# kyoungseoun-chung/pyapes

Hardware: AMD Instinct MI355X
Metric: cell-updates*iters/sec, 3-D Poisson CG (higher is better)
Workload: dtype f64; 1 GPU; 3-D Poisson 512x512x512 double, periodic BCs, CG (BASELINE config 3); global_cells=134217728, parallelism=single

## Files before the change

### pyapes_amd/csrc/pa_bc.hip

```cpp
#include "pa_host.h"

#include <math.h>
#include <stdlib.h>
#include <stdio.h>
#include <string.h>

#include <algorithm>
#include <new>

template <typename T>
struct BCArgs {
  int axis, side, type;
  T sval;
  const T* vals;
  T c23, dxf, ndir;
  T c43, c13;
  const T* far0;
  const T* far1;
  const int* done;
};

template <typename T>
__global__ void __launch_bounds__(PA_BLOCK) k_bc_face(DevGeom G, T* __restrict__ x, BCArgs<T> B) {
  if (B.done && *B.done) return;
// ... 346 lines not shown
    T t1 = B.c43 * x[base + (p1 - off) * st];
    T t2 = B.c13 * x[base + (p2 - off) * st];
    t1 = t1 - t2;
    return t1 + ct;
  }
  if (B.type == 3) return x[base + (p1 - off) * st];
  if (lower) {
    T vp = x[base + (1 - off) * st];
    T vf = B.far0 ? B.far0[q] : x[base + (N - 1 - off) * st];
    T vff = B.far0 ? B.far1[q] : x[base + (N - 2 - off) * st];
    T t1 = vp - vf;
    return t1 + vff;
  }
  if (B.far0) {
    T t1 = B.far0[q] - x[base + (N - 1 - off) * st];
    return t1 + x[base + (N - 2 - off) * st];
  }
  return x0_new;
}

template <typename T>
__global__ void __launch_bounds__(PA_BLOCK) k_bc_pair(DevGeom G, T* __restrict__ x, BCPairArgs<T> P,
                                                       const int* __restrict__ done, T* __restrict__ shell_old,
                                                       double* __restrict__ partials, int mode) {
  if (done && *done) return;
  const int a = P.axis;
  const int64_t nu = (a == 0) ? G.n1 : G.n0;
  const int64_t nv = (a == 2) ? G.n1 : G.n2;
  const int64_t N = (a == 0) ? G.g0 : (a == 1 ? G.n1 : G.n2);
  const int64_t off = (a == 0) ? G.off0 : 0;
  const int64_t st = (a == 0) ? G.s0 : (a == 1 ? G.s1 : 1);
  double s[1] = {0.0};
  for (int64_t q = (int64_t)blockIdx.x * blockDim.x + threadIdx.x; q < nu * nv;
       q += (int64_t)gridDim.x * blockDim.x) {
    const int64_t u = q / nv, v = q - u * nv;
    int64_t base;
    bool owned = true;
    if (a == 0) {
      base = u * G.s1 + v;
      if (G.act[1] && (u == 0 || u == G.n1 - 1)) owned = false;
      if (G.act[2] && (v == 0 || v == G.n2 - 1)) owned = false;
    } else if (a == 1) {
      base = u * G.s0 + v;
      if (G.act[2] && (v == 0 || v == G.n2 - 1)) owned = false;
    } else {
      base = u * G.s0 + v * G.s1;
    }
    T x0_new = (T)0;
    if (P.lo.type) {
      T* xf = x + base + (0 - off) * st;
      T val;
      if (mode == 3) {
        val = *xf;
      } else {
        val = pa_bc_face_value<T>(P.lo, x, base, st, off, N, q, (T)0);
        *xf = val;
      }
      x0_new = val;
// ... 13 lines not shown
      T val;
      if (mode == 3) {
        val = *xf;
      } else {
        val = pa_bc_face_value<T>(P.hi, x, base, st, off, N, q, x0_new);
        *xf = val;
      }
      if (mode && owned) {
        if (mode == 1) {
          T df = val - shell_old[P.pos_hi + q];
          T p = df * df;
          s[0] += (double)p;
        }
        shell_old[P.pos_hi + q] = val;
      }
    }
  }
  if (mode == 1) pa_block_reduce_store<1>(s, partials);
}

template <typename T>
static int pa_bc_shell_fused(pa_ctx* c, T* x, double* part2, int with_delta, bool guarded, int* nsh, bool standalone);
template <typename T>
static int pa_bc_pair_apply(pa_ctx* c, T* x, double* part2, int mode, bool guarded, int* nsh);
template <typename T>
static void pa_shell_launch(pa_ctx* c, const T* x, T* shell, double* part2, int with_delta);

template <typename T>
int pa_bc_apply_faces(pa_ctx* c, T* x, bool guarded) {
  const DevGeom& G = c->G;
  for (int w = 0; w < c->nbc; ++w) {
    int f = c->bc_order[w];
    const HostBC& b = c->bc[f];
    if (b.type == PA_BC_NONE) continue;
    int a = f >> 1, side = f & 1;
    if (!G.act[a]) continue;
    if (a == 0) {
      if (side == 0 && G.off0 != 0) continue;
      if (side == 1 && G.off0 + G.n0 != G.g0) continue;
    }
    BCArgs<T> B;
    memset(&B, 0, sizeof(B));
    B.axis = a; B.side = side; B.type = b.type;
    B.vals = (const T*)b.vals;
    B.c43 = (T)(4.0 / 3.0);
    B.c13 = (T)(1.0 / 3.0);
    B.c23 = (T)(2.0 / 3.0);
// ... 199 lines not shown
    if (side == 0 && G.off0 != 0) B.type = 0;
    if (side == 1 && G.off0 + G.n0 != G.g0) B.type = 0;
  }
  B.vals = (const T*)b.vals;
  B.c43 = (T)(4.0 / 3.0);
  B.c13 = (T)(1.0 / 3.0);
  B.c23 = (T)(2.0 / 3.0);
  B.dxf = (T)b.dxf;
  B.ndir = side == 0 ? (T)-1 : (T)1;
  B.done = guarded ? pa_done_flag(c) : nullptr;
  if (b.type == PA_BC_DIRICHLET) B.sval = (T)b.value;
  if (b.type == PA_BC_NEUMANN) {
    T pre = (T)((2.0 / 3.0) * b.value);
    pre = pre * B.dxf;
    pre = pre * B.ndir;
    B.sval = pre;
  }
  if (b.type == PA_BC_PERIODIC && a == 0 && G.n0 != G.g0) {
    B.far0 = (const T*)(side == 0 ? c->bc_far_lo0 : c->bc_far_hi0);
    B.far1 = (const T*)c->bc_far_lo1;
  }
}

template <typename T>
static int pa_bc_pair_apply(pa_ctx* c, T* x, double* part2, int mode, bool guarded, int* nsh) {
  const DevGeom& G = c->G;
  const int64_t sz[3] = {G.n1 * G.n2, G.n0 * G.n2, G.n0 * G.n1};
  int64_t start[6], total = 0;
  for (int f = 0; f < 6; ++f) { start[f] = total; total += G.act[f >> 1] ? sz[f >> 1] : 0; }
  T* shell = (T*)c->scr[SCR_SHELL];
  int rows = 0;
  for (int a = 0; a < 3; ++a) {
    if (!G.act[a]) continue;
    BCPairArgs<T> P;
    bc_face_args<T>(c, 2 * a, P.lo, guarded);
    bc_face_args<T>(c, 2 * a + 1, P.hi, guarded);
    if (mode != 3 && ((P.lo.type == PA_BC_PERIODIC && a == 0 && G.n0 != G.g0 && !P.lo.far0) ||
                      (P.hi.type == PA_BC_PERIODIC && a == 0 && G.n0 != G.g0 && !P.hi.far0))) {
      pa_set_err(c, "periodic axis-0 BC on a slab needs the far planes (pa_slab_set)");
      return PA_E_STATE;
    }
    if (!P.lo.type && !P.hi.type) continue;
    P.axis = a;
    P.pos_lo = start[2 * a];
    P.pos_hi = start[2 * a + 1];
    const int nb = pa_grid_blocks(sz[a]);
    hipLaunchKernelGGL(k_bc_pair<T>, dim3(nb), dim3(PA_BLOCK), 0, c->stream, G, x, P,
                       guarded ? pa_done_flag(c) : (const int*)nullptr, shell, part2 ? part2 + rows : nullptr,
                       mode);
    if (mode == 1) rows += nb;
  }
  if (nsh) *nsh = rows;
  PA_HIP(c, hipGetLastError());
  return PA_OK;
}


int pa_bc_shell_rows(const pa_ctx* c) {
  if (c->bc_fused || !c->bc_pair) return pa_shell_blocks(c);
  const DevGeom& G = c->G;
  const int64_t sz[3] = {G.n1 * G.n2, G.n0 * G.n2, G.n0 * G.n1};
  int rows = 0;
  for (int a = 0; a < 3; ++a) {
    if (!G.act[a]) continue;
    int lo = c->bc[2 * a].type, hi = c->bc[2 * a + 1].type;
    if (a == 0) {
      if (G.off0 != 0) lo = 0;
      if (G.off0 + G.n0 != G.g0) hi = 0;
    }
    if (lo || hi) rows += pa_grid_blocks(sz[a]);
  }
  return rows;
}

template <typename T>
static void pa_shell_launch(pa_ctx* c, const T* x, T* shell, double* part2, int with_delta) {
  hipLaunchKernelGGL(k_shell<T>, dim3(pa_shell_blocks(c)), dim3(PA_BLOCK), 0, c->stream, c->G, c->sc, x, shell, part2,
                     with_delta);
}

void pa_bc_plan(pa_ctx* c) {
  c->bc_static = pa_bc_is_static(c);
  c->bc_fused = pa_bc_fusable(c);
  c->bc_pair = (!c->bc_fused && pa_bc_pairable(c)) ? 1 : 0;
  c->shell_cur = 0;
}

template <typename T>
int pa_bc_fill_start(pa_ctx* c, T* x, bool filled_by_driver) {
  if (c->bc_fused && !filled_by_driver)
    return pa_bc_shell_fused<T>(c, x, nullptr, 0, false, nullptr, false);
  if (c->bc_pair) return pa_bc_pair_apply<T>(c, x, nullptr, filled_by_driver ? 3 : 2, false, nullptr);
  if (!filled_by_driver)
    if (int rc = pa_bc_apply_faces<T>(c, x)) return rc;
  pa_shell_launch<T>(c, (const T*)x, (T*)c->scr[SCR_SHELL], (double*)c->scr[SCR_PART2], 0);
  return PA_OK;
}

template <typename T>
int pa_bc_fill_step(pa_ctx* c, T* x, double* part2, int* nsh) {
  *nsh = 0;
  if (c->bc_static) return PA_OK;
  if (c->bc_fused) return pa_bc_shell_fused<T>(c, x, part2, 1, true, nsh, false);
  if (c->bc_pair) return pa_bc_pair_apply<T>(c, x, part2, 1, true, nsh);
  if (int rc = pa_bc_apply_faces<T>(c, x, true)) return rc;
  *nsh = pa_shell_blocks(c);
  pa_shell_launch<T>(c, (const T*)x, (T*)c->scr[SCR_SHELL], part2, 1);
  return PA_OK;
}

#define PA_BC_INST(T)                                                                            \
  template int pa_bc_apply_faces<T>(pa_ctx*, T*, bool);                                          \
  template int pa_bc_apply_auto<T>(pa_ctx*, T*, bool);                                           \
  template int pa_bc_fill_start<T>(pa_ctx*, T*, bool);                                           \
  template int pa_bc_fill_step<T>(pa_ctx*, T*, double*, int*);
PA_BC_INST(float)
PA_BC_INST(double)
#undef PA_BC_INST
```

### pyapes_amd/csrc/pa_cg3d.hip

```cpp
#include "pa_cg3d_kernel.h"
#include "pa_cg2d_kernel.h"

template <typename T>
int pa_cg3d_phase_a(pa_ctx* c, const DevEq<T>& E, Vec<T> r, Vec<T> d, T* dnew, double* partials) {
  const int mode = c->cg_pitch ? 3 : cg3d_mode<T>(c, E, {r.p, d.p, dnew, r.glo, r.ghi, d.glo, d.ghi}, false, false, true);
  if (!mode) return 0;
  const bool rz = c->coord == PA_COORD_RZ;
  Cg3dArgs<T> A;
  memset(&A, 0, sizeof(A));
  fill_common<T>(c, E, A);
  A.ps1 = c->cg_ps1; A.ps0 = c->cg_ps1 * c->G.n1;
  A.r = r; A.d = d; A.dnew = dnew; A.partials = partials;
  A.reverse = 0;
  if (c->fold_b_n > 0) {
    A.pre_part = c->fold_b_part;
    A.pre_n = c->fold_b_n;
    A.pre_shell = c->fold_b_shell ? c->fold_b_shell : (const double*)c->scr[SCR_PART2];
    A.pre_nsh = c->fold_b_nsh;
    A.sc_w = c->sc_alt;
    A.pre_sums = pa_sums(c);
  }
  int n = (mode == 1 || mode == 3 || mode == 4) ? launch_cg2d<T, 0>(c, A, mode == 3) : 0;
  if (n == 0 && rz) return 0;
  if (n == 0) n = launch_any<T, 0>(c, A, mode);
// ... 7 lines not shown
}

template <typename T>
int pa_cg3d_phase_b(pa_ctx* c, const DevEq<T>& E, Vec<T> d, T* x, T* r, double* partials) {
  T* const r_out = c->cg_r_out ? (T*)c->cg_r_out : r;
  const int mode = c->cg_pitch ? 3 : cg3d_mode<T>(c, E, {d.p, x, r, r_out, d.glo, d.ghi, c->r_send_lo, c->r_send_hi}, false, false, true);
  if (!mode) return 0;
  const bool rz = c->coord == PA_COORD_RZ;
  Cg3dArgs<T> A;
  memset(&A, 0, sizeof(A));
  fill_common<T>(c, E, A);
  A.ps1 = c->cg_ps1; A.ps0 = c->cg_ps1 * c->G.n1;
  A.d = d; A.x = x; A.rw = r; A.rw_out = r_out; A.partials = partials;
  if (!c->slab_fold_live) {
    A.send_lo = (T*)c->r_send_lo; A.send_hi = (T*)c->r_send_hi;
  }
  A.reverse = 1;
  if (c->fold_a_n > 0) {
    A.pre_part = (const double*)c->scr[SCR_PART] + 2 * (size_t)PA_MAX_PARTIALS;
    A.pre_n = c->fold_a_n;
    A.sc_w = c->sc;
    A.pre_sums = pa_sums(c);
  }
  int n = (mode == 1 || mode == 3 || mode == 4) ? launch_cg2d<T, 1>(c, A, mode == 3) : 0;
  if (n == 0 && rz) return 0;
  if (n == 0) n = launch_any<T, 1>(c, A, mode);
  if (n > 0 && hipGetLastError() != hipSuccess) { pa_set_err(c, "k_cg3d phase B launch failed"); return PA_E_HIP; }
  if (n > 0) c->fold_a_n = 0;
  return n;
}

template <typename T>
int pa_tile3d_jacobi(pa_ctx* c, const DevEq<T>& E, Vec<T> x, const T* rhs, T* xnew, double omega, double* partials) {
  const int mode = cg3d_mode<T>(c, E, {x.p, rhs, xnew, x.glo, x.ghi}, false, false, true);
  if (!mode) return 0;
  const bool rz = c->coord == PA_COORD_RZ;
  Cg3dArgs<T> A;
  memset(&A, 0, sizeof(A));
  fill_common<T>(c, E, A);
  A.d = x; A.out = xnew; A.aux = rhs; A.p0 = (T)omega; A.partials = partials;
  if (c->fold_b_n > 0) {
    A.pre_part = c->fold_b_part;
    A.pre_n = c->fold_b_n;
    A.pre_shell = c->fold_b_shell ? c->fold_b_shell : (const double*)c->scr[SCR_PART2];
    A.pre_nsh = c->fold_b_nsh;
    A.sc_w = c->sc_alt;
    A.pre_sums = pa_sums(c);
  }
  int n = 0;
  if (mode == 1 || mode == 4) {
    const bool back2 = c->jac_alt && c->jac_dir && !c->plan_only;
// ... 25 lines not shown
```

### pyapes_amd/csrc/pa_cg3d_kernel.h

```cpp
#pragma once
#include "pa_host.h"

#include <stdio.h>
#include <stdlib.h>
#include <string.h>

template <typename T> struct VecOf;
template <> struct VecOf<double> { static constexpr int N = 2; typedef double type __attribute__((ext_vector_type(2))); };
template <> struct VecOf<float>  { static constexpr int N = 4; typedef float type __attribute__((ext_vector_type(4))); };

template <typename T>
struct Cg3dArgs {
  DevGeom G;
  LapCoef<T> lap;
  T coeff, sign;
  int has_coeff;
  const T* coeff_f;
  const SolverScalars* sc;
  Vec<T> r, d;
  T* dnew;
  T* x;
  T* rw;
  T* rw_out;
  T* send_lo;
// ... 10 lines not shown
  int lap_off;
  GradCoef<T> grd;
  int gnd;
  int64_t ps0, ps1;
  const T* rz;
  int64_t rz_n;
  int interior_only;
  int out_all;
  int bcl_type[6];
  T bcl_val[6];
  T bcl_c43, bcl_c13;
  const double* pre_part;
  const double* pre_shell;
  int pre_n, pre_nsh;
  SolverScalars* sc_w;
  double* pre_sums;
  const T* stg_phi0;
  T stg_c0, stg_c1;
  const T* src;
  T src_val;
  const T* vel_f[3];
  T vel_v[3];
  int vel_own;
};

__device__ __forceinline__ int pa_xcd_remap(int b, int nb) {
  const int q = nb >> 3, r = nb & 7, xcd = b & 7, w = b >> 3;
  return (xcd < r ? xcd * (q + 1) : r * (q + 1) + (xcd - r) * q) + w;
}

__device__ __forceinline__ int64_t pa_wrapmod(int64_t v, int64_t n) {
  v %= n;
  return v < 0 ? v + n : v;
}

template <typename T, int RJ, int PHASE, bool CF = false, int KIND = 0, int LAY = 0, bool STG = false>
__global__ void __launch_bounds__(256) k_cg3d(Cg3dArgs<T> A) {
  static_assert(!STG || PHASE == 3, "STG: the explicit Euler step");
  constexpr int PH = PHASE == 9 ? 4 : PHASE;
  constexpr bool NARROW = LAY == 1, PITCH = LAY == 2;
  static_assert(!PITCH || ((PH == 0 || PH == 1 || PH == 5 || PH == 6 || PH == 8) && !CF && KIND == 0),
                "PITCH: the CG / BiCGSTAB phases of a plain Laplacian");
  constexpr int VEC = NARROW ? 1 : VecOf<T>::N;
  typedef T V __attribute__((ext_vector_type(VEC)));
  constexpr int TJ = 4 * RJ, TK = 64 * VEC, TKP = TK + 2 * VEC;
  __shared__ __attribute__((aligned(16))) T tile[2][TJ + 2][TKP];

  (void)sizeof(int[PH >= 0 && PH <= 8 ? 1 : -1]);
  T beta = (T)0, alpha = (T)0;
  T omega = (T)0;
  const DevGeom& G = A.G;
  const int lane = threadIdx.x & 63, wv = threadIdx.x >> 6;
  const int vb = pa_xcd_remap(blockIdx.x, gridDim.x);
  const int tiles = A.tiles_j * A.tiles_k;
  const int chunk = vb / tiles, tl = vb - chunk * tiles;
  const int tjb = tl / A.tiles_k, tkb = tl - tjb * A.tiles_k;
  const int64_t i0 = (int64_t)chunk * G.n0 / A.chunks, i1 = (int64_t)(chunk + 1) * G.n0 / A.chunks;
  const int CI = (int)(i1 - i0);
  const int64_t j0 = (int64_t)tjb * TJ, k0 = (int64_t)tkb * TK;
  constexpr int rev = (PHASE == 1 || PHASE == 9) ? 1 : 0;

  const int64_t kg = k0 + (int64_t)lane * VEC;
  const int64_t kc = pa_wrapmod(kg, G.n2);
  const bool kvalid = kg < G.n2;
  const int64_t fs0 = PITCH ? A.ps0 : G.s0, fs1 = PITCH ? A.ps1 : G.s1;
  const int64_t kcf = PITCH ? (kg < fs1 ? kg : 0) : kc;
  int64_t jrow[RJ];
  unsigned rowS = 0, rowShell = 0, rowValid = 0, rowLo = 0, rowHi = 0;
#pragma unroll
  for (int jj = 0; jj < RJ; ++jj) {
    const int64_t jg = j0 + wv * RJ + jj;
    jrow[jj] = pa_wrapmod(jg, G.n1);
    const bool valid = jg < G.n1;
    if (valid) rowValid |= 1u << jj;
    if (valid && jg >= G.slo[1] && jg <= G.shi[1]) rowS |= 1u << jj;
    if (jg == 0 || jg == G.n1 - 1) rowShell |= 1u << jj;
    const int rc = pa_row_case(G, 1, jg, G.n1, G.treat);
    if (rc == 1) rowLo |= 1u << jj;
    if (rc == 2) rowHi |= 1u << jj;
  }
  unsigned rowPLo = 0, rowPHi = 0, colPLo = 0, colPHi = 0;
  if (PH == 3 || PH == 7 || KIND != 0) {
#pragma unroll
    for (int jj = 0; jj < RJ; ++jj) {
      const int64_t jg = j0 + wv * RJ + jj;
      if (G.bct[2] == 4 && jg == 1) rowPLo |= 1u << jj;
      if (G.bct[3] == 4 && jg == G.n1 - 2) rowPHi |= 1u << jj;
    }
#pragma unroll
    for (int v = 0; v < VEC; ++v) {
      if (G.bct[4] == 4 && kg + v == 1) colPLo |= 1u << v;
      if (G.bct[5] == 4 && kg + v == G.n2 - 2) colPHi |= 1u << v;
    }
  }
  unsigned colS = 0, colShell = 0, colLo = 0, colHi = 0;
#pragma unroll
  for (int v = 0; v < VEC; ++v) {
    const int64_t kk = kg + v;
    if (kvalid && kk >= G.slo[2] && kk <= G.shi[2]) colS |= 1u << v;
    if (kk == 0 || kk == G.n2 - 1) colShell |= 1u << v;
    const int rc = pa_row_case(G, 2, kk, G.n2, G.treat);
    if (rc == 1) colLo |= 1u << v;
    if (rc == 2) colHi |= 1u << v;
  }
#ifdef PA_PLAIN_EXPERIMENT
  rowLo = rowHi = colLo = colHi = 0;
  rowS = rowValid = (1u << RJ) - 1;
  colS = (1u << VEC) - 1;
#endif
  const int64_t hrow = (wv == 0) ? pa_wrapmod(j0 - 1, G.n1) : pa_wrapmod(j0 + TJ, G.n1);
  const bool hvec = (wv == 0 || wv == 3);
  const bool hsc = (wv == 1 && lane < 2 * TJ);
  const int hs_row = lane >> 1, hs_side = lane & 1;
  const int64_t hs_off = pa_wrapmod(j0 + hs_row, G.n1) * fs1 +
                         (hs_side ? pa_wrapmod(k0 + TK, G.n2) : pa_wrapmod(k0 - 1, G.n2));

  auto plane_of = [&](int q) -> int64_t { return rev ? (i1 - 1 - q) : (i0 + q); };
  auto pptr = [&](const Vec<T>& v, int64_t ii) -> const T* {
    return ii < 0 ? v.glo : (ii >= G.n0 ? v.ghi : v.p + ii * fs0);
  };

  struct Raw {
    V d[RJ];
    V r[RJ];
    V q[RJ];
    V hd, hr, hq;
// ... 650 lines not shown
        } else if (PH == 0) {
          const T e = inS ? xc : (T)0;
          outd[v] = e;
          T p = e * res[jj][v];
          s0 += (double)p;
        } else {
          const T xo = xv[jj][v];
          T ad = alpha * xc;
          T xn = xo + ad;
          T aAd = alpha * res[jj][v];
          T rn = rv[jj][v] - aAd;
          xn = inS ? xn : xo;
          rn = inS ? rn : (T)0;
          T p = rn * rn;
          s0 += (double)p;
          const bool offshell = inS && !(iShell || (rowShell >> jj & 1) || (colShell >> v & 1));
          T df = xn - xo;
          T p2 = df * df;
          s1 += offshell ? (double)p2 : 0.0;
          outd[v] = rn;
          outx[v] = xn;
        }
      }
      if (kvalid && (rowValid >> jj & 1)) {
        const int64_t o = ii * G.s0 + jrow[jj] * G.s1 + kc;
        const int64_t ob = PITCH ? ii * fs0 + jrow[jj] * fs1 + kcf : o;
        if (PH == 8) {
          *reinterpret_cast<V*>(A.out2 + ob) = outx;
        } else if (PH == 5 || PH == 6) {
          if (PH == 5 || A.out) *reinterpret_cast<V*>(A.out + ob) = outd;
          *reinterpret_cast<V*>(A.out2 + ob) = outx;
        } else if (PH >= 2) {
          *reinterpret_cast<V*>(A.out + o) = outd;
        } else if (PH == 0) {
          if (PITCH) __builtin_nontemporal_store(outd, reinterpret_cast<V*>(A.dnew + ii * fs0 + jrow[jj] * fs1 + kcf));
          else if (NARROW) *reinterpret_cast<V*>(A.dnew + o) = outd;
          else __builtin_nontemporal_store(outd, reinterpret_cast<V*>(A.dnew + o));
        } else {
          if (PITCH) {
            __builtin_nontemporal_store(outd, reinterpret_cast<V*>(A.rw_out + ii * fs0 + jrow[jj] * fs1 + kcf));
            T* xp = A.x + ii * G.s0 + jrow[jj] * G.s1;
#pragma unroll
            for (int v = 0; v < VEC; ++v)
              if (kg + v < G.n2) xp[kg + v] = outx[v];
          } else if (NARROW) {
            *reinterpret_cast<V*>(A.x + o) = outx;
// ... 70 lines not shown
  if (c->ndim != 3 && c->ndim != 2) return 0;
  int il, id;
  if (!eq_lap_div<T>(E, il, id, field_speed) || (id >= 0 && !allow_div)) return 0;
  if ((c->ndim == 3 && c->G.n0 < 3) || c->G.n1 < 3 || c->G.n2 < 3) return 0;
  uintptr_t bits = il >= 0 ? (uintptr_t)E.t[il].coeff_f : 0;
  if (id >= 0) bits |= (uintptr_t)E.t[id].u_f;
  for (const void* q : ptrs) bits |= (uintptr_t)q;
  if (bits & (sizeof(T) - 1)) return 0;
  constexpr int VEC = VecOf<T>::N;
  if ((bits & 15) || c->G.n2 % VEC != 0 || c->G.n2 < 2 * VEC) return 2;
  return 1;
}

static int cus_of(pa_ctx* c) {
  static int cus = 0;
  if (!cus) {
    hipDeviceProp_t prop;
    if (hipGetDeviceProperties(&prop, c->device) == hipSuccess) cus = prop.multiProcessorCount;
    if (cus <= 0) cus = 256;
  }
  return cus;
}

template <typename T, int RJ, int PHASE, bool CF, int KIND = 0, int LAY = 0, bool STG = false>
static int blocks_per_cu() {
  static int cached = 0;
  if (!cached) {
    int n = 0;
    if (hipOccupancyMaxActiveBlocksPerMultiprocessor(&n, k_cg3d<T, RJ, PHASE, CF, KIND, LAY, STG>, 256, 0) != hipSuccess || n <= 0) n = 2;
    cached = n;
  }
  return cached;
}

template <typename T, int RJ, int PHASE, bool CF = false, int KIND = 0, int LAY = 0, bool STG = false>
static int launch_cg3d(pa_ctx* c, Cg3dArgs<T>& A) {
  constexpr bool NARROW = LAY == 1;
  constexpr int VEC = NARROW ? 1 : VecOf<T>::N;
  constexpr int TJ = 4 * RJ, TK = 64 * VEC;
  const DevGeom& G = c->G;
  int64_t n1e = G.n1, n2e = G.n2;
  if (PHASE == 0 || PHASE == 1 || PHASE == 5 || PHASE == 6 || PHASE == 8) {
    if (G.bct[3] != PA_BC_PERIODIC && n1e > 2) n1e -= 1;
    if (G.bct[5] != PA_BC_PERIODIC && n2e > 2) n2e -= 1;
  }
  A.tiles_j = (int)((n1e + TJ - 1) / TJ);
  A.tiles_k = (int)((n2e + TK - 1) / TK);
  const int tiles = A.tiles_j * A.tiles_k;
  const int capacity = cus_of(c) * blocks_per_cu<T, RJ, PHASE, CF, KIND, LAY, STG>();
  int chunks = capacity / tiles;
  if (chunks < 1) chunks = 1;
  if (chunks > G.n0) chunks = (int)G.n0;
  if (c->chunks > 0 && chunks > c->chunks) chunks = c->chunks;
  A.chunks = chunks;
  const int nblk = tiles * chunks;
  if (nblk > PA_MAX_PARTIALS) return 0;
  static int dbg = -1;
  if (dbg < 0) dbg = getenv("PYAPES_HIP_DEBUG") ? 8 : 0;
  if (dbg > 0) {
    --dbg;
    fprintf(stderr, "[pyapes_hip] k_cg3d phase %c%s%s: tiles %dx%d chunks %d (CI ~%lld) blocks %d, %d blocks/CU x %d CUs\n",
            (char)('A' + PHASE), LAY == 1 ? " (narrow)" : (LAY == 2 ? " (pitched)" : ""), STG ? " (RK stage)" : "", A.tiles_j, A.tiles_k, chunks, (long long)(G.n0 / chunks), nblk,
            blocks_per_cu<T, RJ, PHASE, CF, KIND, LAY, STG>(), cus_of(c));
  }
  if (c->plan_only) return nblk;
  hipLaunchKernelGGL((k_cg3d<T, RJ, PHASE, CF, KIND, LAY, STG>), dim3(nblk), dim3(256), 0, c->stream, A);
  return nblk;
}

template <typename T, int PHASE = 0>
static int pick_rj(pa_ctx* c, bool narrow = false, bool cg_phase = false) {
  const int VEC = narrow ? 1 : VecOf<T>::N;
  const DevGeom& G = c->G;
  if (!G.act[0]) return 4;
  const int64_t n1e = G.n1 - ((cg_phase && G.bct[3] != PA_BC_PERIODIC && G.n1 > 2) ? 1 : 0);
  const int64_t n2e = G.n2 - ((cg_phase && G.bct[5] != PA_BC_PERIODIC && G.n2 > 2) ? 1 : 0);
  const int64_t tk = (n2e + 64 * VEC - 1) / (64 * VEC);
  const int cap = cus_of(c) * 2;
  auto chunk_len = [&](int rj) {
    const int64_t tiles = ((n1e + 4 * rj - 1) / (4 * rj)) * tk;
    const int64_t chunks = cap / tiles > 0 ? cap / tiles : 1;
    return G.n0 / chunks;
  };
  if (PHASE == 3) {
    return chunk_len(4) >= 12 ? 4 : 2;
  }
  if (G.n1 <= 4) return 1;
  if (G.n1 <= 8) return 2;
  return (chunk_len(4) < 24 && chunk_len(2) >= 24) ? 2 : 4;
// ... 26 lines not shown
      PA_EULER_CASE(PA_OP_DIV_UPWIND_COMPAT)
      PA_EULER_CASE(PA_OP_DIV_UPWIND)
      default: return 0;
    }
#undef PA_EULER_CASE
  }
  if constexpr (PHASE == 2 || PHASE == 5 || PHASE == 6 || PHASE == 8) {
    if (A.kind != 0) {
      const bool four = pick_rj<T>(c, NARROW == 1) == 4;
#define PA_DIV_CASE(K)                                                                   \
      case K:                                                                            \
        return four ? launch_cg3d<T, 4, PHASE, false, K, NARROW>(c, A)                   \
                    : launch_cg3d<T, 2, PHASE, false, K, NARROW>(c, A);
      switch (A.kind) {
        PA_DIV_CASE(PA_OP_DIV_CENTRAL)
        PA_DIV_CASE(PA_OP_DIV_UPWIND_COMPAT)
        PA_DIV_CASE(PA_OP_DIV_UPWIND)
        default: return 0;
      }
#undef PA_DIV_CASE
    }
  }
  const int rj = pick_rj<T>(c, NARROW == 1, PHASE == 0 || PHASE == 1 || PHASE == 5 || PHASE == 6 || PHASE == 8);
  switch (rj) {
    case 1: return launch_cg3d<T, 1, PHASE, false, 0, NARROW>(c, A);
    case 2: return launch_cg3d<T, 2, PHASE, false, 0, NARROW>(c, A);
    default: return launch_cg3d<T, 4, PHASE, false, 0, NARROW>(c, A);
  }
}

template <typename T, int PHASE>
static int launch_pitched(pa_ctx* c, Cg3dArgs<T>& A) {
  static_assert(PHASE == 0 || PHASE == 1 || PHASE == 5 || PHASE == 6 || PHASE == 8, "PITCH: CG / BiCGSTAB phases");
  if (A.coeff_f || A.kind != 0) return 0;
  switch (pick_rj<T>(c, false, true)) {
    case 1: return launch_cg3d<T, 1, PHASE, false, 0, 2>(c, A);
    case 2: return launch_cg3d<T, 2, PHASE, false, 0, 2>(c, A);
    default: return launch_cg3d<T, 4, PHASE, false, 0, 2>(c, A);
  }
}

template <typename T, int PHASE, bool STG = false>
static int launch_any(pa_ctx* c, Cg3dArgs<T>& A, int mode) {
  if constexpr (PHASE == 0 || PHASE == 1 || PHASE == 5 || PHASE == 6 || PHASE == 8) {
    if (mode == 3) return launch_pitched<T, PHASE>(c, A);
  }
// ... 41 lines not shown
```

### pyapes_amd/csrc/pa_core.hip

```cpp
#include "pa_host.h"

#include <dlfcn.h>
#include <math.h>
#include <stdlib.h>
#include <stdio.h>
#include <string.h>

#include <algorithm>
#include <chrono>
#include <new>

template <typename T>
__global__ void __launch_bounds__(PA_BLOCK) k_rz_tables(int64_t nr, const T* __restrict__ r_nodes, T dr,
                                                         T* __restrict__ tab) {
  auto nn = [](T v) -> T { return (isnan(v) || isinf(v)) ? (T)0 : v; };
  const T h2 = dr * dr;
  const T c23 = (T)(2.0 / 3.0), c13 = (T)(1.0 / 3.0);
  for (int64_t i = (int64_t)blockIdx.x * blockDim.x + threadIdx.x; i < nr; i += (int64_t)gridDim.x * blockDim.x) {
    const T r = r_nodes[i];
    T t = (T)2 * r;
    const T s = nn(dr / t);
    T ap = (T)1 + s;
    T am = (T)1 - s;
    tab[i] = ap / h2;
// ... 267 lines not shown

int pa_ctx_set_option(pa_ctx* c, const char* name, int value) {
  if (!c || !name) return PA_E_ARG;
  if (c->solve != PA_SOLVE_NONE) { pa_set_err(c, "pa_ctx_set_option during a solve"); return PA_E_STATE; }
  if (!strcmp(name, "fastpath")) c->fastpath = value != 0;
  else if (!strcmp(name, "sf")) c->sf = (value == 2 || value == 4) ? value : (value != 0);
  else if (!strcmp(name, "chunks")) c->chunks = value < 0 ? 0 : value;
  else if (!strcmp(name, "vself")) c->vself = value != 0;
  else if (!strcmp(name, "sfq")) c->sfq = value < 0 ? 0 : value;
  else if (!strcmp(name, "fold")) c->fold = value != 0;
  else if (!strcmp(name, "resident")) c->resident = value != 0;
  else if (!strcmp(name, "cg2d_mincells")) c->cg2d_mincells = value;
  else if (!strcmp(name, "bcl")) c->bcl = value != 0;
  else if (!strcmp(name, "pitch")) c->pitch = value != 0;
  else if (!strcmp(name, "place")) c->place = value != 0;
  else if (!strcmp(name, "place_minbytes")) c->ps.minbytes = value < 0 ? 0 : (size_t)value;
  else if (!strcmp(name, "place_blocks")) c->ps.blocks = value < 0 ? 0 : (value > PA_PLACE_MAXSPARE ? PA_PLACE_MAXSPARE : value);
  else if (!strcmp(name, "place_budget")) c->ps.budget = 0.01 * (value < 0 ? 0 : value);
  else if (!strcmp(name, "resident_coop")) c->resident_coop = value != 0;
  else if (!strcmp(name, "bc_path")) c->bc_path = value & 7;
  else if (!strcmp(name, "bicg_pfold")) c->bicg_pfold = value != 0;
  else if (!strcmp(name, "bicg_srv")) c->bicg_srv = value != 0;
  else if (!strcmp(name, "jac_alt")) c->jac_alt = value != 0;
  else if (!strcmp(name, "rhs_full")) c->rhs_full = value != 0;
  else if (!strcmp(name, "res_cells")) c->res_cells = value;
  else if (!strcmp(name, "res_nt")) c->res_nt = value;
  else if (!strcmp(name, "res_nt_cells")) c->res_nt_cells = value;
  else if (!strcmp(name, "res_spin")) c->res_spin = value;
  else if (!strcmp(name, "res_rzlean")) c->res_rzlean = value != 0;
  else if (!strcmp(name, "comm")) c->opt_comm = value != 0;
  else if (!strcmp(name, "slab_fold")) c->opt_slab_fold = value != 0;
  else if (!strcmp(name, "comm_overlap")) c->comm_overlap = value < 0 ? -1 : (value != 0);
  else if (!strcmp(name, "comm_timeout")) c->comm_timeout = value > 0 ? value : 60;
  else if (!strcmp(name, "roctx")) { g_roctx.want = value != 0; g_roctx.state = 0; }
  else { pa_set_err(c, "pa_ctx_set_option: unknown option '%s'", name); return PA_E_ARG; }
  return PA_OK;
}

int pa_ctx_get_option(const pa_ctx* c, const char* name, int* value) {
  if (!c || !name || !value) return PA_E_ARG;
  const struct { const char* n; int v; } tab[] = {
      {"fastpath", c->fastpath}, {"sf", c->sf}, {"sfq", c->sfq}, {"vself", c->vself}, {"chunks", c->chunks}, {"fold", c->fold}, {"resident", c->resident}, {"bcl", c->bcl}, {"pitch", c->pitch},
      {"place", c->place}, {"resident_coop", c->resident_coop}, {"bc_path", c->bc_path}, {"bicg_pfold", c->bicg_pfold}, {"bicg_srv", c->bicg_srv}, {"jac_alt", c->jac_alt},
      {"rhs_full", c->rhs_full}, {"comm", c->opt_comm}, {"slab_fold", c->opt_slab_fold}, {"comm_overlap", c->comm_overlap},
      {"comm_timeout", c->comm_timeout}, {"place_blocks", c->ps.blocks}};
  for (const auto& t : tab)
    if (!strcmp(name, t.n)) { *value = t.v; return PA_OK; }
  return PA_E_ARG;
}

int pa_ctx_destroy(pa_ctx* c) {
  if (!c) return PA_OK;
  (void)hipSetDevice(c->device);
  (void)hipStreamSynchronize(c->stream);
  if (c->comm) (void)pa_comm_destroy(c);
  pa_place_destroy(c);
  for (int q = 0; q < PA_NSCRATCH; ++q)
    if (c->scr_base[q]) (void)hipFree(c->scr_base[q]);
  if (c->sc_base) (void)hipFree(c->sc_base);
  if (c->sums) (void)hipFree(c->sums);
  if (c->rows_buf[0]) (void)hipFree(c->rows_buf[0]);
  if (c->rows_buf[1]) (void)hipFree(c->rows_buf[1]);
  if (c->h_sc) (void)hipHostFree(c->h_sc);
  for (int q = 0; q < 2; ++q) {
    if (c->h_poll[q]) (void)hipHostFree(c->h_poll[q]);
    if (c->ev_poll[q]) (void)hipEventDestroy(c->ev_poll[q]);
// ... 163 lines not shown
```

### pyapes_amd/csrc/pa_host.h

```cpp
#pragma once
#include <hip/hip_runtime.h>
#include <stdarg.h>
#include <stdint.h>

#include "../../include/pyapes_hip.h"
#include "pa_device.h"

#define PA_MAX_GRID 2048
#define PA_MAX_PARTIALS 131072

struct SolverScalars {
  double rr, rr_old, dAd, alpha, beta, tol, tolerance;
  double rho, omega, rho_next, r0v, ts, tt, r0t;
  long long itr, max_it;
  int done, err, finished_early;
};

struct HostBC {
  int type = PA_BC_NONE;
  double value = 0.0;
  const void* vals = nullptr;
  double dxf = 0.0;
};

// ... 75 lines not shown
  double* sums = nullptr;
  double* ext_sums = nullptr;
  hipEvent_t ev0 = nullptr, ev1 = nullptr;
  hipEvent_t ev_switch = nullptr;
  PaSolve solve = PA_SOLVE_NONE;
  int cur = 0, pending_init_logic = 0, b_blocks = 0;
  int bc_static = 0, bc_fused = 0, bc_pair = 0;
  int shell_cur = 0;
  void* cg_x = nullptr;
  const void* jac_rhs = nullptr;
  double jac_omega = 1.0;
  void* cg_r_out = nullptr;
  int64_t cg2d_mincells = 1500000;
  int bcl = 1;
  int place = 1;
  PlaceSearch ps;
  int pitch = 1;
  int bc_path = 0;
  int bicg_pfold = 1;
  int bicg_srv = 1;
  int bicg_s_stored = 1;
  int jac_alt = 1;
  int jac_dir = 0;
  int rhs_full = 0;
  int res_cells = 0, res_nt = 0, res_nt_cells = 0, res_spin = -1, res_rzlean = 1;
  int opt_comm = 1;
  int opt_slab_fold = 1;
  int comm_overlap = -1;
  int comm_timeout = 60;
  int cg_pitch = 0;
  int64_t cg_ps1 = 0;
  void* x_old_out = nullptr;
  int slab = 0;
  const void* x_glo = nullptr;
  const void* x_ghi = nullptr;
  void* r_send_lo = nullptr;
  void* r_send_hi = nullptr;
  const void* r_recv_lo = nullptr;
  const void* r_recv_hi = nullptr;
  void* d_glo[2] = {nullptr, nullptr};
  void* d_ghi[2] = {nullptr, nullptr};
  const void* bc_far_lo0 = nullptr;
  const void* bc_far_lo1 = nullptr;
  const void* bc_far_hi0 = nullptr;
  void* v_send_lo = nullptr;
  void* v_send_hi = nullptr;
// ... 26 lines not shown
};

static inline double* pa_sums(const pa_ctx* c) { return (c->slab && c->ext_sums) ? c->ext_sums : c->sums; }

static inline const int* pa_done_flag(const pa_ctx* c) { return &c->sc->done; }

void pa_set_err(pa_ctx* c, const char* fmt, ...);
void pa_range_push(const char* name);
void pa_range_pop();
struct PaRange {
  explicit PaRange(const char* name) { pa_range_push(name); }
  ~PaRange() { pa_range_pop(); }
};
int pa_hip_fail(pa_ctx* c, hipError_t e, const char* what);
int pa_grid_blocks(int64_t work);
int pa_scratch(pa_ctx* c, void** slot, size_t* cap, size_t bytes);
void pa_refresh_geom(pa_ctx* c);
int pa_bc_apply_any(pa_ctx* c, void* x);
int pa_check_eq_applicable(pa_ctx* c);
int pa_check_div_kind(pa_ctx* c, int kind, const char* who = "pa_div");
int pa_require_solve(pa_ctx* c, PaSolve kind, const char* what);
int pa_cg_slab_mid(pa_ctx* c);
int pa_cg_slab_flush(pa_ctx* c);
int pa_bc_shell_rows(const pa_ctx* c);
void pa_profile_stop(pa_ctx* c, int which);
int pa_place_begin(pa_ctx* c, const void* x, size_t array_bytes);
int pa_place_tick(pa_ctx* c);
int pa_place_batch_end(pa_ctx* c);
void pa_place_r_written(pa_ctx* c);
int pa_place_prepare_block(pa_ctx* c, void* block);
void pa_place_end(pa_ctx* c, int may_free);
void pa_place_reset(pa_ctx* c);
void pa_place_destroy(pa_ctx* c);

int pa_shell_blocks(const pa_ctx* c);
int64_t pa_shell_elems(const pa_ctx* c);
bool pa_bc_is_static(const pa_ctx* c);
bool pa_bc_fusable(const pa_ctx* c);
bool pa_bc_pairable(const pa_ctx* c);
template <typename T>
int pa_bc_apply_faces(pa_ctx* c, T* x, bool guarded = false);
template <typename T>
int pa_bc_apply_auto(pa_ctx* c, T* x, bool guarded);
void pa_bc_plan(pa_ctx* c);
template <typename T>
int pa_bc_fill_start(pa_ctx* c, T* x, bool filled_by_driver);
// ... 60 lines not shown
```

### pyapes_amd/hip/context.py

```python
from __future__ import annotations

import ctypes as C
import warnings
from typing import Any, Sequence

import torch
from torch import Tensor

from ..backend import require_gpu
from . import lib as L


def _check(ctx: "HipContext | None", lib: C.CDLL, rc: int, handle: Any = None) -> None:
    if rc == L.PA_OK:
        return
    msg = lib.pa_last_error(handle).decode() if lib is not None else "?"
    raise L.PaError(rc, msg)


class HipContext:
    def __init__(self, mesh: Any):
        if not mesh.is_cuda or not torch.cuda.is_available():
            raise RuntimeError(
                "pyapes_amd: a HIP context needs a mesh on device='cuda' and a visible MI355X; "
# ... 448 lines not shown
        self._rc(rc)
        return rep

    def report(self) -> L.PaReport:
        rep = L.PaReport()
        self._rc(self.lib.pa_report_read(self.h, C.byref(rep)))
        return rep

    def scalars(self) -> dict[str, float]:
        v = (C.c_double * 16)()
        self._rc(self.lib.pa_scalars_read(self.h, v))
        names = ("alpha", "beta", "rr", "rr_old", "dAd", "tol", "rho", "omega", "rho_next", "r0v", "ts", "tt", "r0t", "itr")
        return {n: float(v[i]) for i, n in enumerate(names)}

    def place_stats(self) -> dict[str, float]:
        v = (C.c_double * 10)()
        self._rc(self.lib.pa_place_stats(self.h, v))
        names = ("state", "trials", "kept", "allocations", "spent_us", "timed_us", "best_pair_us", "blocks_held",
                 "first_pair_us", "passes_done")
        out = {n: float(v[i]) for i, n in enumerate(names)}
        out["state"] = {-1: "off", 0: "idle", 1: "searching", 2: "done"}[int(v[0])]
        return out

    def profile(self, on: bool) -> None:
        self._rc(self.lib.pa_profile_set(self.h, int(on)))

    def profile_read(self) -> dict[str, float]:
        ma, mb = C.c_double(), C.c_double()
        na, nb = C.c_int64(), C.c_int64()
        self._rc(self.lib.pa_profile_read(self.h, C.byref(ma), C.byref(na), C.byref(mb), C.byref(nb)))
        return {"phase_a_ms": ma.value / max(na.value, 1), "phase_a_n": na.value,
                "phase_b_ms": mb.value / max(nb.value, 1), "phase_b_n": nb.value}

    def comm_unique_id(self) -> bytes:
        buf = C.create_string_buffer(128)
        rc = self.lib.pa_comm_unique_id(C.cast(buf, C.c_void_p))
        if rc != L.PA_OK:
            raise L.PaError(rc, "pa_comm_unique_id: librccl not available")
        return buf.raw

    def comm_available(self) -> bool:
        return bool(self.lib.pa_comm_available())

    def comm_size(self) -> int:
        n = C.c_int(0)
        self._rc(self.lib.pa_comm_count(self.h, C.byref(n)))
# ... 115 lines not shown
```

Baseline: 87.25 billion cell-updates*iters/s.

## Fuse periodic z-face BC fill into CG phase B kernel via lane shuffles

When z is periodic and the row is exactly one wavefront of vectors wide, the phase-B CG kernel shifts its k tiles by half a tile. It then computes the periodic z ghost values in-register with readlane, writes them, and adds their delta-squared into the residual sum. The separate BC pair kernel then only processes a thin frame of rows near the x/y edges on the z faces, instead of the full z-face plane. This cuts the extra memory traffic of the z-face BC pass. In exchange it adds a second template variant with a different occupancy bound, extra per-row register work, and host-side state tracking that guards against mixing the two paths in the middle of a solve.

Result: no change. 87.13 billion cell-updates*iters/s (-0.1%).

```diff
diff --git a/pyapes_amd/csrc/pa_bc.hip b/pyapes_amd/csrc/pa_bc.hip
--- a/pyapes_amd/csrc/pa_bc.hip
+++ b/pyapes_amd/csrc/pa_bc.hip
@@ -392,7 +392,7 @@
 template <typename T>
 __global__ void __launch_bounds__(PA_BLOCK) k_bc_pair(DevGeom G, T* __restrict__ x, BCPairArgs<T> P,
                                                        const int* __restrict__ done, T* __restrict__ shell_old,
-                                                       double* __restrict__ partials, int mode) {
+                                                       double* __restrict__ partials, int mode, int frame) {
   if (done && *done) return;
   const int a = P.axis;
   const int64_t nu = (a == 0) ? G.n1 : G.n0;
@@ -401,9 +401,21 @@
   const int64_t off = (a == 0) ? G.off0 : 0;
   const int64_t st = (a == 0) ? G.s0 : (a == 1 ? G.s1 : 1);
   double s[1] = {0.0};
-  for (int64_t q = (int64_t)blockIdx.x * blockDim.x + threadIdx.x; q < nu * nv;
-       q += (int64_t)gridDim.x * blockDim.x) {
-    const int64_t u = q / nv, v = q - u * nv;
+  const int64_t fw = frame, work = fw ? nu * nv - (nu - 2 * fw) * (nv - 2 * fw) : nu * nv;
+  for (int64_t t = (int64_t)blockIdx.x * blockDim.x + threadIdx.x; t < work;
+       t += (int64_t)gridDim.x * blockDim.x) {
+    int64_t u, v;
+    if (!fw) {
+      u = t / nv; v = t - u * nv;
+    } else if (t < 2 * fw * nv) {
+      u = t / nv; v = t - u * nv;
+      if (u >= fw) u += nu - 2 * fw;
+    } else {
+      const int64_t m = t - 2 * fw * nv, w = m % (2 * fw);
+      u = fw + m / (2 * fw);
+      v = w < fw ? w : nv - 2 * fw + w;
+    }
+    const int64_t q = u * nv + v;
     int64_t base;
     bool owned = true;
     if (a == 0) {
@@ -463,7 +475,7 @@
 template <typename T>
 static int pa_bc_shell_fused(pa_ctx* c, T* x, double* part2, int with_delta, bool guarded, int* nsh, bool standalone);
 template <typename T>
-static int pa_bc_pair_apply(pa_ctx* c, T* x, double* part2, int mode, bool guarded, int* nsh);
+static int pa_bc_pair_apply(pa_ctx* c, T* x, double* part2, int mode, bool guarded, int* nsh, bool zframe = false);
 template <typename T>
 static void pa_shell_launch(pa_ctx* c, const T* x, T* shell, double* part2, int with_delta);
 
@@ -709,8 +721,12 @@
   }
 }
 
-template <typename T>
-static int pa_bc_pair_apply(pa_ctx* c, T* x, double* part2, int mode, bool guarded, int* nsh) {
+static int64_t pa_zframe_rows(const DevGeom& G) {
+  return G.n0 * G.n1 - (G.n0 - 2 * PA_ZFRAME) * (G.n1 - 2 * PA_ZFRAME);
+}
+
+template <typename T>
+static int pa_bc_pair_apply(pa_ctx* c, T* x, double* part2, int mode, bool guarded, int* nsh, bool zframe) {
   const DevGeom& G = c->G;
   const int64_t sz[3] = {G.n1 * G.n2, G.n0 * G.n2, G.n0 * G.n1};
   int64_t start[6], total = 0;
@@ -731,10 +747,11 @@
     P.axis = a;
     P.pos_lo = start[2 * a];
     P.pos_hi = start[2 * a + 1];
-    const int nb = pa_grid_blocks(sz[a]);
+    const int frame = (a == 2 && zframe) ? PA_ZFRAME : 0;
+    const int nb = pa_grid_blocks(frame ? pa_zframe_rows(G) : sz[a]);
     hipLaunchKernelGGL(k_bc_pair<T>, dim3(nb), dim3(PA_BLOCK), 0, c->stream, G, x, P,
                        guarded ? pa_done_flag(c) : (const int*)nullptr, shell, part2 ? part2 + rows : nullptr,
-                       mode);
+                       mode, frame);
     if (mode == 1) rows += nb;
   }
   if (nsh) *nsh = rows;
@@ -755,7 +772,7 @@
       if (G.off0 != 0) lo = 0;
       if (G.off0 + G.n0 != G.g0) hi = 0;
     }
-    if (lo || hi) rows += pa_grid_blocks(sz[a]);
+    if (lo || hi) rows += pa_grid_blocks((a == 2 && c->zwrap_filled) ? pa_zframe_rows(G) : sz[a]);
   }
   return rows;
 }
@@ -771,6 +788,7 @@
   c->bc_fused = pa_bc_fusable(c);
   c->bc_pair = (!c->bc_fused && pa_bc_pairable(c)) ? 1 : 0;
   c->shell_cur = 0;
+  c->zwrap_filled = c->zwrap_stale = 0;
 }
 
 template <typename T>
@@ -789,7 +807,16 @@
   *nsh = 0;
   if (c->bc_static) return PA_OK;
   if (c->bc_fused) return pa_bc_shell_fused<T>(c, x, part2, 1, true, nsh, false);
-  if (c->bc_pair) return pa_bc_pair_apply<T>(c, x, part2, 1, true, nsh);
+  if (c->bc_pair) {
+    const bool zframe = c->zwrap_filled != 0;
+    c->zwrap_filled = 0;
+    if (zframe) c->zwrap_stale = 1;
+    if (!zframe && c->zwrap_stale) {
+      pa_set_err(c, "BC fill: the tiled CG phase B stopped filling the z faces in the middle of a solve");
+      return PA_E_STATE;
+    }
+    return pa_bc_pair_apply<T>(c, x, part2, 1, true, nsh, zframe);
+  }
   if (int rc = pa_bc_apply_faces<T>(c, x, true)) return rc;
   *nsh = pa_shell_blocks(c);
   pa_shell_launch<T>(c, (const T*)x, (T*)c->scr[SCR_SHELL], part2, 1);
diff --git a/pyapes_amd/csrc/pa_cg3d.hip b/pyapes_amd/csrc/pa_cg3d.hip
--- a/pyapes_amd/csrc/pa_cg3d.hip
+++ b/pyapes_amd/csrc/pa_cg3d.hip
@@ -53,11 +53,19 @@
     A.sc_w = c->sc;
     A.pre_sums = pa_sums(c);
   }
+  const bool zwrap = c->zwrap && mode == 1 && !A.coeff_f && c->ndim == 3 && c->coord == PA_COORD_XYZ && !c->slab && !c->cg_pitch &&
+                     c->G.n2 == 64 * VecOf<T>::N && c->bc[4].type == PA_BC_PERIODIC &&
+                     c->bc[5].type == PA_BC_PERIODIC && c->bc_pair && !c->bc_static && c->G.n0 >= 7 && c->G.n1 >= 7;
+  A.zwrap = zwrap ? 1 : 0;
   int n = (mode == 1 || mode == 3 || mode == 4) ? launch_cg2d<T, 1>(c, A, mode == 3) : 0;
   if (n == 0 && rz) return 0;
   if (n == 0) n = launch_any<T, 1>(c, A, mode);
   if (n > 0 && hipGetLastError() != hipSuccess) { pa_set_err(c, "k_cg3d phase B launch failed"); return PA_E_HIP; }
   if (n > 0) c->fold_a_n = 0;
+  if (n > 0 && zwrap && !c->plan_only) {
+    c->zwrap_filled = 1;
+    ++c->zwrap_fills;
+  }
   return n;
 }
 
diff --git a/pyapes_amd/csrc/pa_cg3d_kernel.h b/pyapes_amd/csrc/pa_cg3d_kernel.h
--- a/pyapes_amd/csrc/pa_cg3d_kernel.h
+++ b/pyapes_amd/csrc/pa_cg3d_kernel.h
@@ -56,7 +56,16 @@
   const T* vel_f[3];
   T vel_v[3];
   int vel_own;
+  int zwrap;
 };
+
+__device__ __forceinline__ double pa_lane_value(double v, int l) {
+  const int lo = __builtin_amdgcn_readlane(__double2loint(v), l), hi = __builtin_amdgcn_readlane(__double2hiint(v), l);
+  return __hiloint2double(hi, lo);
+}
+__device__ __forceinline__ float pa_lane_value(float v, int l) {
+  return __int_as_float(__builtin_amdgcn_readlane(__float_as_int(v), l));
+}
 
 __device__ __forceinline__ int pa_xcd_remap(int b, int nb) {
   const int q = nb >> 3, r = nb & 7, xcd = b & 7, w = b >> 3;
@@ -68,8 +77,9 @@
   return v < 0 ? v + n : v;
 }
 
-template <typename T, int RJ, int PHASE, bool CF = false, int KIND = 0, int LAY = 0, bool STG = false>
-__global__ void __launch_bounds__(256) k_cg3d(Cg3dArgs<T> A) {
+template <typename T, int RJ, int PHASE, bool CF = false, int KIND = 0, int LAY = 0, bool STG = false, bool ZW = false>
+__global__ void __launch_bounds__(256, ZW ? 2 : 1) k_cg3d(Cg3dArgs<T> A) {
+  static_assert(!ZW || (PHASE == 1 && LAY == 0 && !CF), "ZW: CG phase B, vector layout, scalar coefficient");
   static_assert(!STG || PHASE == 3, "STG: the explicit Euler step");
   constexpr int PH = PHASE == 9 ? 4 : PHASE;
   constexpr bool NARROW = LAY == 1, PITCH = LAY == 2;
@@ -91,7 +101,8 @@
   const int tjb = tl / A.tiles_k, tkb = tl - tjb * A.tiles_k;
   const int64_t i0 = (int64_t)chunk * G.n0 / A.chunks, i1 = (int64_t)(chunk + 1) * G.n0 / A.chunks;
   const int CI = (int)(i1 - i0);
-  const int64_t j0 = (int64_t)tjb * TJ, k0 = (int64_t)tkb * TK;
+  constexpr bool zw = ZW;
+  const int64_t j0 = (int64_t)tjb * TJ, k0 = (int64_t)tkb * TK - (zw ? TK / 2 : 0);
   constexpr int rev = (PHASE == 1 || PHASE == 9) ? 1 : 0;
 
   const int64_t kg = k0 + (int64_t)lane * VEC;
@@ -130,12 +141,23 @@
   unsigned colS = 0, colShell = 0, colLo = 0, colHi = 0;
 #pragma unroll
   for (int v = 0; v < VEC; ++v) {
-    const int64_t kk = kg + v;
+    const int64_t kk = (zw ? kc : kg) + v;
     if (kvalid && kk >= G.slo[2] && kk <= G.shi[2]) colS |= 1u << v;
     if (kk == 0 || kk == G.n2 - 1) colShell |= 1u << v;
     const int rc = pa_row_case(G, 2, kk, G.n2, G.treat);
     if (rc == 1) colLo |= 1u << v;
     if (rc == 2) colHi |= 1u << v;
+  }
+  unsigned rowZ = 0;
+  if constexpr (ZW) {
+    if (tkb == 0) {
+      const int wvu = __builtin_amdgcn_readfirstlane(wv);
+#pragma unroll
+      for (int jj = 0; jj < RJ; ++jj) {
+        const int64_t jg = j0 + wvu * RJ + jj;
+        if (jg >= PA_ZFRAME && jg < G.n1 - PA_ZFRAME) rowZ |= 1u << jj;
+      }
+    }
   }
 #ifdef PA_PLAIN_EXPERIMENT
   rowLo = rowHi = colLo = colHi = 0;
@@ -832,6 +854,22 @@
           outx[v] = xn;
         }
       }
+      if constexpr (ZW) {
+        {
+          const bool fz = (rowZ >> jj & 1) && ii >= PA_ZFRAME && ii < G.n0 - PA_ZFRAME;
+          const T x1 = pa_lane_value(outx[1], 32);
+          const T xf = pa_lane_value(outx[VEC - 1], 31);
+          const T xff = pa_lane_value(outx[VEC - 2], 31);
+          T t1 = x1 - xf;
+          const T z0 = t1 + xff;
+          const bool l31 = fz && lane == 31, l32 = fz && lane == 32;
+          T df = z0 - (l31 ? xv[jj][VEC - 1] : xv[jj][0]);
+          T p2 = df * df;
+          s1 += (l31 || l32) ? (double)p2 : 0.0;
+          outx[VEC - 1] = l31 ? z0 : outx[VEC - 1];
+          outx[0] = l32 ? z0 : outx[0];
+        }
+      }
       if (kvalid && (rowValid >> jj & 1)) {
         const int64_t o = ii * G.s0 + jrow[jj] * G.s1 + kc;
         const int64_t ob = PITCH ? ii * fs0 + jrow[jj] * fs1 + kcf : o;
@@ -948,18 +986,18 @@
   return cus;
 }
 
-template <typename T, int RJ, int PHASE, bool CF, int KIND = 0, int LAY = 0, bool STG = false>
+template <typename T, int RJ, int PHASE, bool CF, int KIND = 0, int LAY = 0, bool STG = false, bool ZW = false>
 static int blocks_per_cu() {
   static int cached = 0;
   if (!cached) {
     int n = 0;
-    if (hipOccupancyMaxActiveBlocksPerMultiprocessor(&n, k_cg3d<T, RJ, PHASE, CF, KIND, LAY, STG>, 256, 0) != hipSuccess || n <= 0) n = 2;
+    if (hipOccupancyMaxActiveBlocksPerMultiprocessor(&n, k_cg3d<T, RJ, PHASE, CF, KIND, LAY, STG, ZW>, 256, 0) != hipSuccess || n <= 0) n = 2;
     cached = n;
   }
   return cached;
 }
 
-template <typename T, int RJ, int PHASE, bool CF = false, int KIND = 0, int LAY = 0, bool STG = false>
+template <typename T, int RJ, int PHASE, bool CF = false, int KIND = 0, int LAY = 0, bool STG = false, bool ZW = false>
 static int launch_cg3d(pa_ctx* c, Cg3dArgs<T>& A) {
   constexpr bool NARROW = LAY == 1;
   constexpr int VEC = NARROW ? 1 : VecOf<T>::N;
@@ -973,7 +1011,7 @@
   A.tiles_j = (int)((n1e + TJ - 1) / TJ);
   A.tiles_k = (int)((n2e + TK - 1) / TK);
   const int tiles = A.tiles_j * A.tiles_k;
-  const int capacity = cus_of(c) * blocks_per_cu<T, RJ, PHASE, CF, KIND, LAY, STG>();
+  const int capacity = cus_of(c) * blocks_per_cu<T, RJ, PHASE, CF, KIND, LAY, STG, ZW>();
   int chunks = capacity / tiles;
   if (chunks < 1) chunks = 1;
   if (chunks > G.n0) chunks = (int)G.n0;
@@ -987,10 +1025,10 @@
     --dbg;
     fprintf(stderr, "[pyapes_hip] k_cg3d phase %c%s%s: tiles %dx%d chunks %d (CI ~%lld) blocks %d, %d blocks/CU x %d CUs\n",
             (char)('A' + PHASE), LAY == 1 ? " (narrow)" : (LAY == 2 ? " (pitched)" : ""), STG ? " (RK stage)" : "", A.tiles_j, A.tiles_k, chunks, (long long)(G.n0 / chunks), nblk,
-            blocks_per_cu<T, RJ, PHASE, CF, KIND, LAY, STG>(), cus_of(c));
+            blocks_per_cu<T, RJ, PHASE, CF, KIND, LAY, STG, ZW>(), cus_of(c));
   }
   if (c->plan_only) return nblk;
-  hipLaunchKernelGGL((k_cg3d<T, RJ, PHASE, CF, KIND, LAY, STG>), dim3(nblk), dim3(256), 0, c->stream, A);
+  hipLaunchKernelGGL((k_cg3d<T, RJ, PHASE, CF, KIND, LAY, STG, ZW>), dim3(nblk), dim3(256), 0, c->stream, A);
   return nblk;
 }
 
@@ -1063,6 +1101,15 @@
     }
   }
   const int rj = pick_rj<T>(c, NARROW == 1, PHASE == 0 || PHASE == 1 || PHASE == 5 || PHASE == 6 || PHASE == 8);
+  if constexpr (PHASE == 1 && NARROW == 0) {
+    if (A.zwrap) {
+      switch (rj) {
+        case 1: return launch_cg3d<T, 1, 1, false, 0, 0, false, true>(c, A);
+        case 2: return launch_cg3d<T, 2, 1, false, 0, 0, false, true>(c, A);
+        default: return launch_cg3d<T, 4, 1, false, 0, 0, false, true>(c, A);
+      }
+    }
+  }
   switch (rj) {
     case 1: return launch_cg3d<T, 1, PHASE, false, 0, NARROW>(c, A);
     case 2: return launch_cg3d<T, 2, PHASE, false, 0, NARROW>(c, A);
diff --git a/pyapes_amd/csrc/pa_core.hip b/pyapes_amd/csrc/pa_core.hip
--- a/pyapes_amd/csrc/pa_core.hip
+++ b/pyapes_amd/csrc/pa_core.hip
@@ -313,6 +313,7 @@
   else if (!strcmp(name, "bicg_pfold")) c->bicg_pfold = value != 0;
   else if (!strcmp(name, "bicg_srv")) c->bicg_srv = value != 0;
   else if (!strcmp(name, "jac_alt")) c->jac_alt = value != 0;
+  else if (!strcmp(name, "zwrap")) c->zwrap = value != 0;
   else if (!strcmp(name, "rhs_full")) c->rhs_full = value != 0;
   else if (!strcmp(name, "res_cells")) c->res_cells = value;
   else if (!strcmp(name, "res_nt")) c->res_nt = value;
@@ -333,6 +334,7 @@
   const struct { const char* n; int v; } tab[] = {
       {"fastpath", c->fastpath}, {"sf", c->sf}, {"sfq", c->sfq}, {"vself", c->vself}, {"chunks", c->chunks}, {"fold", c->fold}, {"resident", c->resident}, {"bcl", c->bcl}, {"pitch", c->pitch},
       {"place", c->place}, {"resident_coop", c->resident_coop}, {"bc_path", c->bc_path}, {"bicg_pfold", c->bicg_pfold}, {"bicg_srv", c->bicg_srv}, {"jac_alt", c->jac_alt},
+      {"zwrap", c->zwrap}, {"zwrap_fills", c->zwrap_fills},
       {"rhs_full", c->rhs_full}, {"comm", c->opt_comm}, {"slab_fold", c->opt_slab_fold}, {"comm_overlap", c->comm_overlap},
       {"comm_timeout", c->comm_timeout}, {"place_blocks", c->ps.blocks}};
   for (const auto& t : tab)
diff --git a/pyapes_amd/csrc/pa_host.h b/pyapes_amd/csrc/pa_host.h
--- a/pyapes_amd/csrc/pa_host.h
+++ b/pyapes_amd/csrc/pa_host.h
@@ -121,6 +121,10 @@
   int bicg_s_stored = 1;
   int jac_alt = 1;
   int jac_dir = 0;
+  int zwrap = 1;
+  int zwrap_filled = 0;
+  int zwrap_stale = 0;
+  int zwrap_fills = 0;
   int rhs_full = 0;
   int res_cells = 0, res_nt = 0, res_nt_cells = 0, res_spin = -1, res_rzlean = 1;
   int opt_comm = 1;
@@ -193,6 +197,7 @@
 int pa_require_solve(pa_ctx* c, PaSolve kind, const char* what);
 int pa_cg_slab_mid(pa_ctx* c);
 int pa_cg_slab_flush(pa_ctx* c);
+static constexpr int PA_ZFRAME = 3;
 int pa_bc_shell_rows(const pa_ctx* c);
 void pa_profile_stop(pa_ctx* c, int which);
 int pa_place_begin(pa_ctx* c, const void* x, size_t array_bytes);
diff --git a/pyapes_amd/hip/context.py b/pyapes_amd/hip/context.py
--- a/pyapes_amd/hip/context.py
+++ b/pyapes_amd/hip/context.py
@@ -494,6 +494,9 @@
         out["state"] = {-1: "off", 0: "idle", 1: "searching", 2: "done"}[int(v[0])]
         return out
 
+    def zwrap_fills(self) -> int:
+        return self.get_option("zwrap_fills")
+
     def profile(self, on: bool) -> None:
         self._rc(self.lib.pa_profile_set(self.h, int(on)))
 
```
